# aapo-kossi/gym-eldorado

Hardware: AMD Instinct MI355X
Metric: env-steps/sec at n_envs=65536, 4 players; bit-exact vs C++ ref (higher is better)
Workload: dtype u8; 1 GPU; C5: 65,536 envs in total over the ranks, 4 players, HARD, n_pieces=3, max_steps=100000, on-device masked sampler over selected_action_masks + step, persistent rollout kernel, every step's AoS outputs stored in HBM; n_envs_total=65536, n_envs_per_gpu=65536, seed=12345, parallelism=env-sharded x1 by index (runner.h:33-38 block split), no collectives

## Files before the change

### gym-eldorado_amd/csrc/cog_engine.hip

```cpp
#include <hip/hip_runtime.h>
#include <algorithm>
#include <cstdlib>
#include <cstring>

#include "cog_engine.h"
#include "cog_tables.h"
#include "cog_rng.h"

#define DEV __device__ __forceinline__

#ifdef COG_STAMPS
DEV unsigned long long stamp_clock() {
  unsigned long long t;
  __builtin_amdgcn_sched_barrier(0);
  asm volatile("s_memtime %0\n\ts_waitcnt lgkmcnt(0)" : "=s"(t) :: "memory");
  __builtin_amdgcn_sched_barrier(0);
  return t;
}
#define STAMP(s, k)                                                                          \
  do {                                                                                       \
    const unsigned long long t_ = stamp_clock();                                             \
    if ((s).stamps && (threadIdx.x & 63) == 0)                                               \
      (s).stamps[((size_t)blockIdx.x * (blockDim.x / 64) + threadIdx.x / 64) * 16 + (k)] = t_; \
  } while (0)
// ... 2972 lines not shown
    const uint32_t meta = g[3].w;
    const bool rec = live && (meta & kMetaValid);
    const int ag = (int)((meta >> 2) & 3u), na = (int)((meta >> 4) & 3u), na1 = (int)((meta >> 6) & 3u);
    if (rec) {
      uint32_t dm = 0;
#pragma unroll
      for (int k = 0; k < 7; k++) {
        if (ne4(dk[k], sel4_of(I, ag, k))) dm |= 1u << k;
#pragma unroll
        for (int p = 0; p < 4; p++) I.d[p][k] = sel4(ag == p, dk[k], I.d[p][k]);
      }
#pragma unroll
      for (int k = 0; k < 7; k++) D.slot[k][l] = sel4_of(I, na1, k);
      PH(6);
#ifndef COG_ABLATE_DUOSTORES
      uint8_t *ob = s.obs + i * COG_OBS_BYTES;
      s.info[i * COG_INFO_BYTES + COG_AGENT_INFO0 + COG_AGENT_INFO_STRIDE * ag] = (uint8_t)(meta >> 8);
      if (meta & kMetaMoved) reinterpret_cast<uint4 *>(s.priv + i)[2] = g[6];
#pragma unroll
      for (int k = 0; k < 3; k++) {
        if (ne4(g[k], shb[k])) reinterpret_cast<uint4 *>(ob + COG_OBS_PHASE)[k] = g[k];
        shb[k] = g[k];
      }
      uint8_t *deck = deck_ptr(s, i, ag);
#pragma unroll
      for (int k = 0; k < 7; k++)
        if ((dm >> k) & 1u) reinterpret_cast<uint4 *>(deck)[k] = dk[k];
      const MBits bs{g[3].x, g[3].y, g[3].z}, ba{g[4].x, g[4].y, g[4].z};
      store_mask_record(reinterpret_cast<uint4 *>(s.sel + i * COG_MASK_BYTES), bs, mask_diff_granules(bs, selb));
      selb = bs;
      store_mask_record(reinterpret_cast<uint4 *>(deck + COG_PD_MASK), ba, mask_diff_granules(ba, selm(stb, ag)));
      setm(stb, ag, ba);
      if (na != ag) {
        const MBits bn{g[5].x, g[5].y, g[5].z};
        store_mask_record(reinterpret_cast<uint4 *>(deck_ptr(s, i, na) + COG_PD_MASK), bn,
                          mask_diff_granules(bn, selm(stb, na)));
        setm(stb, na, bn);
      }
      reinterpret_cast<uint2 *>(av + i * COG_ACTION_BYTES)[0] = make_uint2(g[4].w, g[5].w);
#else
      asm volatile("" ::"v"(g[0].x ^ g[1].y ^ g[2].z ^ g[3].x ^ g[4].y ^ g[5].z ^ g[6].w ^ dm ^ dk[0].x ^ dk[6].w));
#endif
      if (!(meta & kMetaEnded)) {
        const uint32_t agent = meta >> 24;
        if (out & 0xffu) s.done[i] = 0;
        if (((out >> 8) & 0xffu) != agent) s.agent[i] = (uint8_t)agent;
        out = agent << 8;
      }
    }
    PH(13);
    __syncthreads();
    PH(7);
  }
  PH_FLUSH(s_glob);
}

template <int SRC>
__global__ void __launch_bounds__(128) k_env_rollout_duo(DevState s, int steps, uint32_t *__restrict__ rngs,
                                                         uint8_t *__restrict__ actions_out) {
  __shared__ DuoLds D;
  const int role = __builtin_amdgcn_readfirstlane((int)(threadIdx.x >> 6));
  park_list_clear_other(s);
  uid_tab_fill(D.tab);
  if (role == 0) {
#ifndef DUO_NOPRIO
    __builtin_amdgcn_s_setprio(3);
#endif
    duo_stepper<SRC>(D, s, steps, rngs);
  } else {
    duo_storer(D, s, steps, actions_out);
  }
}

constexpr int kTrioRingG = 3;
#ifndef COG_TRIO_DEPTH
#define COG_TRIO_DEPTH 8
#endif
constexpr int kTrioDepth = COG_TRIO_DEPTH;
constexpr int kTrioLead = 4;
#ifndef COG_TRIO_BLAG
#define COG_TRIO_BLAG 2
#endif
constexpr int kTrioBLag = COG_TRIO_BLAG;
enum TrioCnt : int { CNT_REC = 0, CNT_DRAW, CNT_STA, CNT_STB, CNT_PRE, CNT_FIN, CNT_ABORT, kTrioCnts };
constexpr uint32_t kTrioSpinLimit = 1u << 21;
struct TrioLds {
  uint2 img[4][5][64];
  uint4 ring[kTrioDepth][kTrioRingG][64];
  uint32_t srng[kTrioDepth][64];
  uint3 pre[kTrioLead][64];
  uint4 pl[4][64];
  uint4 heads[4][64];
  uint4 stbA[4][64];
  uint32_t wide[64];
  uint32_t flg[64];
  uint32_t cnt[kTrioCnts];
  UidEntry tab[kUidTab];
};
static_assert(sizeof(TrioLds) <= 54613, "three trio workgroups per CU (trio_pad_lds keeps two)");
static_assert((kTrioDepth & (kTrioDepth - 1)) == 0 && kTrioDepth >= 4, "ring slots: a power of two");

struct TrioCnt6 {
  uint32_t rec = 0, draw = 0, sta = 0, stb = 0, pre = 0, fin = 0, abort = 0;
};
DEV void cnt_read(const TrioLds &D, TrioCnt6 &c) {
  uint32_t v[kTrioCnts];
#pragma unroll
  for (int k = 0; k < kTrioCnts; k++) v[k] = __hip_atomic_load(&D.cnt[k], __ATOMIC_RELAXED, __HIP_MEMORY_SCOPE_WORKGROUP);
  __builtin_amdgcn_fence(__ATOMIC_ACQUIRE, "workgroup");
  c.rec = __builtin_amdgcn_readfirstlane(v[CNT_REC]);
  c.draw = __builtin_amdgcn_readfirstlane(v[CNT_DRAW]);
  c.sta = __builtin_amdgcn_readfirstlane(v[CNT_STA]);
  c.stb = __builtin_amdgcn_readfirstlane(v[CNT_STB]);
  c.pre = __builtin_amdgcn_readfirstlane(v[CNT_PRE]);
  c.fin = __builtin_amdgcn_readfirstlane(v[CNT_FIN]);
  c.abort = __builtin_amdgcn_readfirstlane(v[CNT_ABORT]);
}
DEV void cnt_store(TrioLds &D, int k, uint32_t v) {
#ifdef COG_TRIO_FENCE
  if ((threadIdx.x & 63) == 0) __hip_atomic_store(&D.cnt[k], v, __ATOMIC_RELEASE, __HIP_MEMORY_SCOPE_WORKGROUP);
#else
  __builtin_amdgcn_fence(__ATOMIC_RELEASE, "wavefront");
  if ((threadIdx.x & 63) == 0) __hip_atomic_store(&D.cnt[k], v, __ATOMIC_RELAXED, __HIP_MEMORY_SCOPE_WORKGROUP);
  __builtin_amdgcn_fence(__ATOMIC_ACQUIRE, "wavefront");
#endif
}
#ifdef COG_ISSUE_COUNT
DEV void cnt_wait(TrioLds &, TrioCnt6 &, const uint32_t &field, uint32_t v, const DevState &) {
  if (field < v) asm volatile("s_nop 0");
}
#else
DEV void cnt_wait(TrioLds &D, TrioCnt6 &c, const uint32_t &field, uint32_t v, const DevState &s) {
  if (__builtin_expect(field >= v, 1)) return;
  if (c.abort) return;
  for (uint32_t spins = 0;; spins++) {
    cnt_read(D, c);
    if (field >= v || c.abort) return;
    if (spins >= kTrioSpinLimit) {
      if ((threadIdx.x & 63) == 0) {
        atomicOr(&s.status[0], F_SYNC_TIMEOUT);
        atomicAdd(&s.status[1], 1u);
        *s.err = 1u;
        __hip_atomic_store(&D.cnt[CNT_ABORT], 1u, __ATOMIC_RELEASE, __HIP_MEMORY_SCOPE_WORKGROUP);
      }
      c.abort = 1u;
      return;
    }
    __builtin_amdgcn_s_sleep(2);
  }
}
#endif
DEV uint3 pre_pack(const uint4 p, bool jtab) {
  if (!jtab) return make_uint3(p.x, p.y, p.z | p.w << 31);
  uint32_t jt = 0u;
#pragma unroll
  for (int k = 2; k <= 9; k++) {
    const UidEntry e = uid_entry((uint32_t)k);
    jt |= uid_tab_accepted(p.y, e.s, e.m) << (4 * (k - 2));
  }
  return make_uint3(p.x, jt, p.z | p.w << 31);
}

DEV void trio_store_players(const TrioLds &D, const DevState &s, int ne) {
  const int l = (int)(threadIdx.x & 63);
#pragma unroll
  for (int j = 0; j < 4; j++) {
    const int f = j * 64 + l, e = min(f >> 2, ne - 1), q = f & 3;
    reinterpret_cast<uint4 *>(s.priv + e)[4 + q] = D.pl[q][e];
    s.heads[5 * e + 1 + q] = D.heads[q][e];
  }
}

DEV void deck_expand(const uint2 pile[5], uint4 dk[7]) {
  uint32_t d[28];
#pragma unroll
  for (int k = 0; k < 28; k++) d[k] = 0u;
#pragma unroll
  for (int p = 0; p < 5; p++) {
    const int b = 21 * p, q = b >> 2, sh = b & 3;
    const uint32_t lo = pile[p].x, hi = pile[p].y;
    if (sh == 0) {
      d[q] |= lo;
      d[q + 1] |= hi;
    } else {
      d[q] |= lo << (8 * sh);
      d[q + 1] |= __builtin_amdgcn_alignbyte(hi, lo, 4 - sh);
      d[q + 2] |= hi >> (8 * (4 - sh));
    }
  }
#pragma unroll
  for (int k = 0; k < 7; k++) dk[k] = make_uint4(d[4 * k], d[4 * k + 1], d[4 * k + 2], d[4 * k + 3]);
}
DEV bool compact_of(const uint4 dk[7], uint2 pile[5]) {
  uint32_t d[28];
#pragma unroll
  for (int k = 0; k < 7; k++) { d[4 * k] = dk[k].x; d[4 * k + 1] = dk[k].y; d[4 * k + 2] = dk[k].z; d[4 * k + 3] = dk[k].w; }
  uint32_t rest = 0u;
#pragma unroll
  for (int k = 0; k < 28; k++) {
    uint32_t m = 0u;
#pragma unroll
    for (int y = 4 * k; y < 4 * k + 4; y++)
      if (y < 105 && y % 21 >= 8) m |= 0xffu << (8 * (y & 3));
    if (m) rest |= d[k] & m;
  }
#pragma unroll
  for (int p = 0; p < 5; p++) {
    const int b = 21 * p, q = b >> 2, sh = b & 3;
    pile[p].x = sh ? __builtin_amdgcn_alignbyte(d[q + 1], d[q], sh) : d[q];
    pile[p].y = sh ? __builtin_amdgcn_alignbyte(d[q + 2], d[q + 1], sh) : d[q + 1];
  }
  return rest == 0u;
}
DEV uint32_t hand_take(uint2 &h, int c) {
  const uint32_t sh = 8u * (uint32_t)(c & 3);
  const uint32_t w = c < 4 ? h.x : h.y;
  const uint32_t prev = (w >> sh) & 0xffu;
  const uint32_t nw = (w & ~(0xffu << sh)) | (((prev - 1u) & 0xffu) << sh);
  h.x = c < 4 ? nw : h.x;
  h.y = c < 4 ? h.y : nw;
  return prev;
}
DEV bool heads14_zero(const MBits &b) { return (b.w0 >> 22) == 1u && b.w1 == (1u << 12) && b.w2 == 0x204u; }
constexpr uint32_t kMoveShopBits = (0x7fu << 2) | (0x7ffffu << 9);
DEV uint32_t nth_set_bit_iter(uint32_t m, uint32_t j) {
  while (__builtin_amdgcn_ballot_w64(j != 0u)) {
    m = j ? (m & (m - 1u)) : m;
    j = j ? j - 1u : 0u;
  }
  return (uint32_t)(__ffs(m) - 1);
}
DEV bool sample_lean(const MBits &sel, const uint3 &pr, uint32_t &rng, uint32_t &a0, bool jtab, const UidEntry *tab) {
  const uint32_t m0 = sel.w0 & 0x3fffffu, k0 = __popc(m0);
  if (!(pr.x == rng && (pr.z >> 31) == 0u && heads14_zero(sel) && k0 >= 1u && k0 <= 9u)) return false;
  uint32_t j;
  if (jtab) {
    j = k0 >= 2u ? (pr.y >> (4u * (k0 - 2u))) & 15u : 0u;
  } else {
    const UidEntry e0 = tab[k0];
    j = k0 >= 2u ? uid_tab_accepted(pr.y, e0.s, e0.m) : 0u;
  }
  a0 = nth_set_bit_iter(m0, j);
  rng = pr.z;
  return true;
}
DEV uint4 pack_lean_player(uint4 pp, uint32_t n_in_hand, uint32_t n_active, uint32_t steps_taken) {
  pp.y = (pp.y & 0xff0000ffu) | (n_in_hand & 0xffu) << 8 | (n_active & 0xffu) << 16;
  pp.z = (pp.z & 0xffff00ffu) | (steps_taken & 0xffu) << 8;
  return pp;
}
DEV bool lean_player(const uint4 &pp) { return (pp.x | (pp.y & 0xffu)) == 0u; }
DEV void trio_store_private(const DevState &s, size_t i, const RegEnv &R, const MBits &selb) {
  uint4 *pw = reinterpret_cast<uint4 *>(s.priv + i);
  reinterpret_cast<uint3 *>(reinterpret_cast<uint32_t *>(pw) + 1)[0] = make_uint3(R.seed, R.max_steps, R.turn_counter);
  pw[1] = make_uint4(R.g1x, R.g1y, R.in_market, R.flags);
  s.heads[5 * i] = mbits_u4(selb);
}

template <int SRC, bool LAT>
DEV void trio_stepper(TrioLds &D, const DevState &s_glob, int steps, int epw, uint32_t *__restrict__ rngs_glob) {
  const int l = (int)(threadIdx.x & 63);
  const size_t wbase = (size_t)blockIdx.x * epw;
  const DevState s = wave_view(s_glob, wbase);
  const size_t i = (size_t)l;
  const int ne = (int)min((size_t)epw, s_glob.n - wbase);
  uint32_t *__restrict__ rngs = rngs_glob + wbase;
  bool live = l < ne;
  uint32_t park = kParkNone, srng = 0;
  PH_DECL;
  TL(10);
  RegEnv R;
  uint2 cells[4];
  int te1 = -1, te2 = -1;
  int ag = 0, na = 0;
  MBits selb = {0u, 0u, 0u}, stab = selb, stnb = selb;
  constexpr bool lat = LAT;
  uint4 pp = make_uint4(0u, 0u, 0u, 0u);
  uint32_t n_in_hand = 0u, n_active = 0u, steps_taken = 0u;
  uint32_t own = 0u;
  if (live) {
    Snap S;
    load_env(s, i, S);
    regs_env(R, S);
    const uint4 *pv4 = reinterpret_cast<const uint4 *>(s.priv + i);
#pragma unroll
    for (int p = 0; p < 4; p++) {
      D.pl[p][l] = pv4[4 + p];
      cells[p] = reinterpret_cast<const uint2 *>(pv4 + 8)[p];
      D.heads[p][l] = s.heads[5 * i + 1 + p];
    }
    srng = rngs[i];
    ag = (int)R.agent();
    na = (int)next_player((uint32_t)ag, R.n_players());
    pp = D.pl[ag][l];
    n_in_hand = (pp.y >> 8) & 0xffu;
    n_active = (pp.y >> 16) & 0xffu;
    steps_taken = (pp.z >> 8) & 0xffu;
#pragma unroll
    for (int p = 0; p < 4; p++) own |= (cells[p].x & 0xffu) << (8 * p);
    selb = S.sel;
    stab = mbits_of(D.heads[ag][l]);
    stnb = mbits_of(D.heads[na][l]);
  }
  R.tab = D.tab;
  __builtin_amdgcn_s_waitcnt(0);
  TL(15);
  __syncthreads();
  uint2 H = make_uint2(0u, 0u);
  bool lean_p = false, narrow = false;
  if (live) {
    H = D.img[ag][1][l];
    narrow = D.wide[l] == 0u;
    lean_p = narrow && lean_player(pp);
  }
  PH(6);
  TL(11);
  TrioCnt6 cc;
  uint3 pr_next = D.pre[0][l];
  bool have_next = true;
  uint2 pf_hd = make_uint2(0u, 0u);
  uint4 pf_pla = make_uint4(0u, 0u, 0u, 0u), pf_hdn = pf_pla;
  bool pf_ok = false;
  for (int t = 0; t < steps; t++) {
    const int sl = t & (kTrioDepth - 1);
    if (t >= kTrioDepth) {
      cnt_wait(D, cc, cc.sta, (uint32_t)(t - kTrioDepth + 1), s_glob);
      cnt_wait(D, cc, cc.stb, (uint32_t)(t - kTrioDepth + 1), s_glob);
    }
    PH(9);
    if (!have_next) cnt_wait(D, cc, cc.pre, (uint32_t)(t - kTrioLead + 1), s_glob);
    PH(2);
    bool ended = false, finish = false, turn_end = false, stepped = false;
    uint32_t a_play = 0u;
    {
      const uint32_t srng0 = srng;
      uint3 pr = pr_next;
      if (!have_next) pr = D.pre[t & (kTrioLead - 1)][l];
      const uint32_t m0 = selb.w0 & 0x3fffffu, k0 = __popc(m0);
      const bool fast = live && pr.x == srng && (pr.z >> 31) == 0u && heads14_zero(selb) && k0 - 1u < 9u;
      uint32_t j;
      if (LAT) {
        j = (pr.y >> (4u * ((k0 - 2u) & 7u))) & 15u;
      } else {
        const UidEntry e0 = R.tab[k0 & (kUidTab - 1)];
        j = uid_tab_accepted(pr.y, e0.s, e0.m);
      }
      j = fast && k0 >= 2u ? j : 0u;
      const uint32_t a0 = nth_set_bit_iter(m0, j);
      a_play = fast ? a0 : 0u;
      srng = fast ? pr.z : srng;
      bool other = false;
      if (__builtin_amdgcn_ballot_w64(live && !fast) && live && !fast) {
#ifdef COG_ISSUE_COUNT
        other = true;
#else
        uint8_t act[5];
        R.sel = heads_of(selb);
        step_action<SRC>(R, make_uint2(0u, 0u), srng, act);
        a_play = act[0];
        other = ((uint32_t)act[1] | act[2] | act[3] | act[4]) != 0u;
#endif
      }
      other = other || a_play > 8u;
      const bool was_done = R.done() != 0u;
      bool hook = false;
      if (t == s.redo_at) hook = s.redo_env < 0 || (int)(wbase + i) == s.redo_env;
      const bool parks = live && !was_done && (!lean_p || other || hook);
      stepped = live && !was_done && !parks;
      if (__builtin_amdgcn_ballot_w64(parks) && parks) {
        srng = srng0;
#ifndef COG_ISSUE_COUNT
        trio_store_private(s, i, R, selb);
        rngs[i] = srng;
#endif
        if (!lat) D.pl[ag][l] = pack_lean_player(pp, n_in_hand, n_active, steps_taken);
        park = (uint32_t)t | kParkRedo;
        live = false;
      }
      uint32_t phase = R.sh[0] & 0xffu;
      if (phase == COG_PHASE_INACTIVE) phase = COG_PHASE_MOVEMENT;
      if (!lat) steps_taken = stepped ? (steps_taken + 1u) & 0xffu : steps_taken;
      const bool play = stepped && a_play != 0u;
      const int c = (int)((a_play - 1u) & 7u);
      uint2 Hp = H;
      const uint32_t prev = hand_take(Hp, c);
      H = play ? Hp : H;
      const uint32_t bp = 1u << (c + 1);
      selb.w0 = play ? (prev > 1u ? (selb.w0 | bp) : (selb.w0 & ~bp)) : selb.w0;
      if (!lat) {
        n_in_hand = play ? (n_in_hand - 1u) & 0xffu : n_in_hand;
        n_active = play ? (n_active + 1u) & 0xffu : n_active;
        pp.z = play ? (pp.z & ~0xffu) | (uint32_t)c : pp.z;
      }
      const uint32_t nph = phase == COG_PHASE_BUYING ? COG_PHASE_INACTIVE : phase + 1u;
      phase = stepped && !play ? nph : phase;
      turn_end = stepped && phase == COG_PHASE_INACTIVE;
      n_active = turn_end ? 0u : n_active;
      const MBits sel0 = selb;
      selb.w0 = turn_end ? stnb.w0 : selb.w0;
      selb.w1 = turn_end ? stnb.w1 : selb.w1;
      selb.w2 = turn_end ? stnb.w2 : selb.w2;
      stab.w0 = turn_end ? sel0.w0 : stab.w0;
      stab.w1 = turn_end ? sel0.w1 : stab.w1;
      stab.w2 = turn_end ? sel0.w2 : stab.w2;
      stnb.w2 = turn_end ? (stnb.w2 & ~kMoveShopBits) | 0x204u : stnb.w2;
      R.g1y = turn_end ? (R.g1y & ~0xffu) | ((uint32_t)na & 0xffu) : R.g1y;
      R.turn_counter += turn_end ? 1u : 0u;
      R.sh[0] = stepped ? (R.sh[0] & ~0xffu) | phase : R.sh[0];
      finish = turn_end && (COG_HEX_END((own >> (8 * na)) & 0xffu) || R.turn_counter >= R.max_steps);
      R.g1x = finish ? (R.g1x & 0x00ffffffu) | (1u << 24) : R.g1x;
      PH(0);
      ended = live && (was_done || finish);
    }
    uint4(*ring)[64] = D.ring[sl];
    int ag1 = ag, na1 = na;
    if (live) {
      ag1 = (int)R.agent();
      na1 = (int)next_player((uint32_t)ag1, R.n_players());
    }
    const bool tc = live && ag1 != ag;
    const bool slow = tc && !pf_ok;
    if (__builtin_amdgcn_ballot_w64(slow)) {
      const int need = R.n_players() == 3u ? te1 : te2;
      const int needw = slow && need >= 0 ? need : INT32_MIN;
      if (__builtin_amdgcn_ballot_w64(needw >= 0)) {
        int dmin = 5;
#pragma unroll
        for (int d = 4; d >= 1; d--) dmin = __builtin_amdgcn_ballot_w64(needw >= t - d) ? d : dmin;
        PH(4);
        cnt_wait(D, cc, cc.draw, (uint32_t)(t - dmin + 1), s_glob);
        PH(5);
      }
      if (slow) {
        pf_hd = D.img[ag1][1][l];
        pf_pla = D.pl[ag1][l];
        pf_hdn = D.heads[na1][l];
      }
    }
    if (live) {
      if (!lat && (tc || ended)) D.pl[ag][l] = pack_lean_player(pp, n_in_hand, n_active, steps_taken);
      const uint32_t meta = kMetaValid | (uint32_t)ag << 2 | (uint32_t)na << 4 | (uint32_t)na1 << 6 |
                            (ended ? kMetaEnded : 0u) | (stepped ? kMetaStepped : 0u) | (uint32_t)ag1 << 24;
      ring[0][l].x = R.sh[0];
      ring[1][l] = make_uint4(selb.w0, selb.w1, selb.w2, meta);
      ring[2][l] = make_uint4(stab.w0, stab.w1, stab.w2, a_play | (lat ? 0u : (n_active & 0xffu) << 8));
      D.srng[sl][l] = srng;
    } else {
      ring[1][l] = make_uint4(0u, 0u, 0u, 0u);
    }
    cnt_store(D, CNT_REC, (uint32_t)(t + 1));
    have_next = t + 1 < kTrioLead || cc.pre >= (uint32_t)(t + 2 - kTrioLead);
    if (have_next) pr_next = D.pre[(t + 1) & (kTrioLead - 1)][l];
    PH(1);
    if (tc) {
      te2 = te1;
      te1 = t;
      H = pf_hd;
      pp = pf_pla;
      n_in_hand = (pf_pla.y >> 8) & 0xffu;
      n_active = (pf_pla.y >> 16) & 0xffu;
      steps_taken = (pf_pla.z >> 8) & 0xffu;
      lean_p = narrow && lean_player(pf_pla);
      stab = stnb;
      stnb = mbits_of(pf_hdn);
      pf_ok = false;
    }
    if (live && !pf_ok && !ended) {
      const int need = R.n_players() == 3u ? te1 : te2;
      if (need < 0 || cc.draw >= (uint32_t)(need + 1)) {
        const int nn = (int)next_player((uint32_t)na1, R.n_players());
        pf_hd = D.img[na1][1][l];
        pf_pla = D.pl[na1][l];
        pf_hdn = D.heads[nn][l];
        pf_ok = true;
      }
    }
    if (live && ended) {
#ifndef COG_ISSUE_COUNT
      trio_store_private(s, i, R, selb);
      rngs[i] = srng;
#endif
      park = (uint32_t)t | (finish ? kParkFinish : 0u);
      live = false;
    }
    ag = ag1;
    na = na1;
    PH(3);
  }
  TL(12);
  if (live && !lat) D.pl[ag][l] = pack_lean_player(pp, n_in_hand, n_active, steps_taken);
  cnt_store(D, CNT_REC, (uint32_t)steps + 1u);
  uint4 *pw = reinterpret_cast<uint4 *>(s.priv + i);
  if (lat) {
    if (live) {
      reinterpret_cast<uint3 *>(reinterpret_cast<uint32_t *>(pw) + 1)[0] = make_uint3(R.seed, R.max_steps, R.turn_counter);
      s.heads[5 * i] = mbits_u4(selb);
      rngs[i] = srng;
    }
    if (l < ne) s.park[i] = park;
    park_list_push(s_glob, park != kParkNone);
  }
  cnt_wait(D, cc, cc.fin, 3u, s_glob);
  PH(7);
  TL(13);
  const uint32_t fl = D.flg[l];
  if (lat) {
    if (live) pw[1] = make_uint4(R.g1x, R.g1y, R.in_market, R.flags | fl);
    else if (l < ne && fl) reinterpret_cast<uint32_t *>(pw)[7] = R.flags | fl;
  } else {
    if (live) {
      R.flags |= fl;
      trio_store_private(s, i, R, selb);
      rngs[i] = srng;
    } else if (l < ne && fl) {
      reinterpret_cast<uint32_t *>(pw)[7] = R.flags | fl;
    }
    if (l < ne) s.park[i] = park;
    park_list_push(s_glob, park != kParkNone);
  }
  trio_store_players(D, s, ne);
  PH(8);
  TL(14);
  PH_FLUSH(s_glob);
}

template <bool LAT>
DEV void trio_draw_play(TrioLds &D, const DevState &s, int l, bool live, int slot, uint32_t mt, uint32_t w2,
                        uint32_t gx, uint4 &p4, uint2 &h, uint2 &a, uint4 &shb0, uint32_t &infob, bool &te,
                        bool &rec_out, uint32_t &dm, uint32_t &nact) {
  const size_t i = (size_t)l;
  const int ag = (int)((mt >> 2) & 3u);
  const bool valid = live && (mt & kMetaValid);
  const bool rec = valid && (mt & kMetaStepped);
  rec_out = rec;
  te = rec && (int)(mt >> 24) != ag;
  const uint32_t a_play = w2 & 0xffu;
  const bool play = rec && a_play != 0u;
  const int c = (int)((a_play - 1u) & 7u);
  if (LAT) {
    uint4 q = p4;
    uint32_t na = (q.y >> 16) & 0xffu;
    q.z = (q.z & 0xffff00ffu) | (((q.z >> 8) + 1u) & 0xffu) << 8;
    q.y = play ? (q.y & 0xffff00ffu) | ((((q.y >> 8) & 0xffu) - 1u) & 0xffu) << 8 : q.y;
    na = play ? (na + 1u) & 0xffu : na;
    q.z = play ? (q.z & ~0xffu) | (a_play - 1u) : q.z;
    na = te ? 0u : na;
    q.y = (q.y & 0xff00ffffu) | na << 16;
    p4.x = rec ? q.x : p4.x;
    p4.y = rec ? q.y : p4.y;
    p4.z = rec ? q.z : p4.z;
    if (rec) D.pl[ag][l] = p4;
    nact = rec ? na : 0u;
  }
  infob = rec ? (infob & ~(0xffu << (8 * ag))) | ((((infob >> (8 * ag)) + 1u) & 0xffu) << (8 * ag)) : infob;
  uint32_t phase = shb0.x & 0xffu;
  phase = phase == COG_PHASE_INACTIVE ? (uint32_t)COG_PHASE_MOVEMENT : phase;
  const bool mv = play && phase == COG_PHASE_MOVEMENT, buy = play && phase == COG_PHASE_BUYING;
  const uint32_t coin = cardf(kRes2, c);
  uint4 g0 = shb0;
  g0.y = mv ? __float_as_uint((float)cardf(kRes0, c)) : g0.y;
  g0.z = mv ? __float_as_uint((float)cardf(kRes1, c)) : g0.z;
  const float bw = __uint_as_float(g0.w) + (coin > 0 ? (float)coin : 0.5f);
  g0.w = mv ? __float_as_uint((float)coin) : buy ? __float_as_uint(bw) : g0.w;
  g0.y = te ? 0u : g0.y;
  g0.z = te ? 0u : g0.z;
  g0.w = te ? 0u : g0.w;
  g0.x = rec ? gx : g0.x;
  if (valid) {
    reinterpret_cast<uint3 *>(&D.ring[slot][0][l].y)[0] = make_uint3(g0.y, g0.z, g0.w);
    s.info[i * COG_INFO_BYTES + COG_AGENT_INFO0 + COG_AGENT_INFO_STRIDE * ag] = (uint8_t)(infob >> (8 * ag));
    if (ne4(g0, shb0)) reinterpret_cast<uint4 *>(s.obs + i * COG_OBS_BYTES + COG_OBS_PHASE)[0] = g0;
  }
  shb0.x = valid ? g0.x : shb0.x;
  shb0.y = valid ? g0.y : shb0.y;
  shb0.z = valid ? g0.z : shb0.z;
  shb0.w = valid ? g0.w : shb0.w;
  const uint32_t sh = 8u * (uint32_t)(c & 3);
  uint32_t hw = c < 4 ? h.x : h.y, aw = c < 4 ? a.x : a.y;
  hw = (hw & ~(0xffu << sh)) | ((((hw >> sh) - 1u) & 0xffu) << sh);
  aw = (aw & ~(0xffu << sh)) | ((((aw >> sh) + 1u) & 0xffu) << sh);
  const bool lo = c < 4;
  h.x = play && lo ? hw : h.x;
  h.y = play && !lo ? hw : h.y;
  a.x = play && lo ? aw : a.x;
  a.y = play && !lo ? aw : a.y;
  if (play) {
    D.img[ag][1][l] = h;
    D.img[ag][2][l] = a;
  }
  const int bh = COG_DECK_HAND + c, ba = COG_DECK_ACTIVE + c;
  dm = play ? 1u << (bh >> 4) | 1u << (ba >> 4) : 0u;
}

template <bool LAT>
DEV uint32_t trio_drawer(TrioLds &D, const DevState &s_glob, int steps, int epw) {
  PH_DECL;
  TL(14);
  const int l = (int)(threadIdx.x & 63);
  const size_t wbase = (size_t)blockIdx.x * epw;
  const DevState s = wave_view(s_glob, wbase);
  const size_t i = (size_t)l;
  const bool live = l < epw && wbase + (size_t)l < s_glob.n;
  uint32_t rng = 0u;
  bool narrow = true;
  constexpr bool lat = LAT;
  uint4 shb0 = make_uint4(0u, 0u, 0u, 0u);
  uint32_t infob = 0u;
  if (live && !s_glob.cdeck_ok) {
#pragma unroll
    for (int p = 0; p < 4; p++) {
      const uint4 *src = reinterpret_cast<const uint4 *>(deck_ptr(s, i, p));
      uint4 dk[7];
      uint2 pile[5];
#pragma unroll
      for (int k = 0; k < 7; k++) dk[k] = src[k];
      narrow = compact_of(dk, pile) && narrow;
#pragma unroll
      for (int q = 0; q < 5; q++) D.img[p][q][l] = pile[q];
    }
  }
  if (live) {
    rng = reinterpret_cast<const uint32_t *>(s.priv + i)[0];
    infob = reinterpret_cast<const uint32_t *>(s.priv + i)[12];
    shb0 = reinterpret_cast<const uint4 *>(s.obs + i * COG_OBS_BYTES + COG_OBS_PHASE)[0];
  }
  if (!s_glob.cdeck_ok) D.wide[l] = narrow ? 0u : 1u;
  uint32_t flags = 0u;
  __builtin_amdgcn_s_waitcnt(0);
  TL(15);
  __syncthreads();
  PH_RESET;
  TrioCnt6 cc;
  for (int r = 0; r < steps; r += 2) {
    const int nrec = r + 1 < steps ? 2 : 1;
    cnt_wait(D, cc, cc.rec, (uint32_t)(r + nrec), s_glob);
    PH(8);
    if (r + nrec >= steps) TL(11);
    const int slot[2] = {r & (kTrioDepth - 1), (r + 1) & (kTrioDepth - 1)};
    uint32_t dm[2] = {0u, 0u}, nact[2] = {0u, 0u};
    int agj[2] = {0, 0};
    bool te[2] = {false, false}, recj[2] = {false, false};
    const uint32_t mt0 = D.ring[slot[0]][1][l].w, w20 = D.ring[slot[0]][2][l].w, gx0 = D.ring[slot[0]][0][l].x;
    uint32_t mt1 = D.ring[slot[1]][1][l].w;
    const uint32_t w21 = D.ring[slot[1]][2][l].w, gx1 = D.ring[slot[1]][0][l].x;
    if (nrec < 2) mt1 = 0u;
    const int ag0 = (int)((mt0 >> 2) & 3u), ag1 = (int)((mt1 >> 2) & 3u);
    uint4 p0 = make_uint4(0u, 0u, 0u, 0u), p1 = p0;
    if (lat) {
      p0 = D.pl[ag0][l];
      p1 = D.pl[ag1][l];
    }
    uint2 h0 = D.img[ag0][1][l], a0 = D.img[ag0][2][l], h1 = D.img[ag1][1][l], a1 = D.img[ag1][2][l];
    trio_draw_play<lat>(D, s, l, live, slot[0], mt0, w20, gx0, p0, h0, a0, shb0, infob, te[0], recj[0], dm[0], nact[0]);
    agj[0] = ag0;
    if (nrec > 1) {
      if (ag1 == ag0) {
        p1.x = p0.x; p1.y = p0.y; p1.z = p0.z; p1.w = p0.w;
        h1.x = h0.x; h1.y = h0.y;
        a1.x = a0.x; a1.y = a0.y;
      }
      trio_draw_play<lat>(D, s, l, live, slot[1], mt1, w21, gx1, p1, h1, a1, shb0, infob, te[1], recj[1], dm[1], nact[1]);
      agj[1] = ag1;
    }
    PH(7);
    const bool any = te[0] || te[1];
    if (__builtin_amdgcn_ballot_w64(any) && any) {
      const int j = te[1] ? 1 : 0, sl = te[1] ? slot[1] : slot[0], ag = te[1] ? agj[1] : agj[0];
      uint2 pile[5];
#pragma unroll
      for (int q = 0; q < 5; q++) pile[q] = D.img[ag][q][l];
      uint4 dk[7], old[7];
      deck_expand(pile, dk);
#pragma unroll
      for (int k = 0; k < 7; k++) old[k] = dk[k];
      const uint4 x = D.ring[sl][2][l];
      MBits ba{x.x, x.y, x.z};
      duo_turn_end(D, l, ag, dk, ba, rng, flags);
      D.ring[sl][2][l] = make_uint4(ba.w0, ba.w1, ba.w2, x.w);
      uint32_t dd = 0;
#pragma unroll
      for (int k = 0; k < 7; k++) dd |= ne4(dk[k], old[k]) ? 1u << k : 0u;
      (void)compact_of(dk, pile);
#pragma unroll
      for (int q = 0; q < 5; q++) D.img[ag][q][l] = pile[q];
      dm[0] |= j == 0 ? dd : 0u;
      dm[1] |= j == 1 ? dd : 0u;
    }
#pragma unroll
    for (int j = 0; j < 2; j++)
      if (j < nrec) {
        uint32_t *w = &D.ring[slot[j]][2][l].w;
        if (lat && recj[j]) *w = (*w & 0xffu) | nact[j] << 8 | dm[j] << 16;
        else reinterpret_cast<uint16_t *>(w)[1] = (uint16_t)dm[j];
      }
    cnt_store(D, CNT_DRAW, (uint32_t)(r + nrec));
    PH(9);
  }
  TL(12);
  if (live) {
    reinterpret_cast<uint32_t *>(s.priv + i)[0] = rng;
    reinterpret_cast<uint32_t *>(s.priv + i)[12] = infob;
  }
  PH_FLUSH(s_glob);
  return flags;
}

template <int PART, bool LAT>
DEV uint32_t trio_storer(TrioLds &D, const DevState &s_glob, int steps, int epw, const uint32_t *__restrict__ rngs_glob,
                         uint8_t *__restrict__ actions_glob) {
  PH_DECL;
  TL(14);
  const int l = (int)(threadIdx.x & 63);
  const size_t wbase = (size_t)blockIdx.x * epw;
  const DevState s = wave_view(s_glob, wbase);
  const size_t i = (size_t)l;
  const bool live = l < epw && wbase + (size_t)l < s_glob.n;
  uint8_t *__restrict__ av = actions_glob + wbase * COG_ACTION_BYTES;
  MBits selb = {0u, 0u, 0u};
  uint2 cells[4];
  uint32_t out = ~0u;
  RegEnv E;
  E.flags = 0u;
  E.avail = 0u;
  uint32_t x = 1u;
  if (live) {
    if (PART == 0) {
      const uint4 *sh4 = reinterpret_cast<const uint4 *>(s.obs + i * COG_OBS_BYTES + COG_OBS_PHASE);
      const uint4 sh1 = sh4[1], sh2 = sh4[2];
      const uint4 *pv4 = reinterpret_cast<const uint4 *>(s.priv + i);
#pragma unroll
      for (int p = 0; p < 4; p++) {
        D.stbA[p][l] = s.heads[5 * i + 1 + p];
        cells[p] = reinterpret_cast<const uint2 *>(pv4 + 8)[p];
      }
      const uint4 g1 = pv4[1];
      const uint32_t w[5] = {sh1.x, sh1.y, sh1.z, sh1.w, sh2.x};
      E.avail = shop_avail_of(w, (g1.y >> 8) & 0xffu, g1.z);
      if (s_glob.cdeck_ok) {
        const uint4 *src = s.cdeck + 10 * i;
        uint4 c[10];
#pragma unroll
        for (int g = 0; g < 10; g++) c[g] = src[g];
#pragma unroll
        for (int g = 0; g < 10; g++) {
          D.img[(2 * g) / 5][(2 * g) % 5][l] = make_uint2(c[g].x, c[g].y);
          D.img[(2 * g + 1) / 5][(2 * g + 1) % 5][l] = make_uint2(c[g].z, c[g].w);
        }
      }
    } else {
      selb = mbits_of(s.heads[5 * i]);
      x = rngs_glob[wbase + (size_t)l];
    }
  }
  if (PART == 0 && s_glob.cdeck_ok) D.wide[l] = live ? s.cwide[i] : 0u;
  if (PART == 1) {
#pragma unroll
    for (int k = 0; k < kTrioLead; k++) {
      const uint4 p = presample(x);
      D.pre[k][l] = pre_pack(p, LAT);
      x = p.z;
    }
  }
  __builtin_amdgcn_s_waitcnt(0);
  TL(15);
  __syncthreads();
  PH_RESET;
  constexpr int LAG = PART == 1 ? kTrioBLag : 0;
  auto deck_rec = [&](int q) {
    const int sl = q & (kTrioDepth - 1);
    const uint32_t meta = D.ring[sl][1][l].w;
    const int ag = (int)((meta >> 2) & 3u);
    if (live && (meta & kMetaValid)) {
      const uint32_t dm = D.ring[sl][2][l].w >> 16;
      uint2 pile[5];
#pragma unroll
      for (int k = 0; k < 5; k++) pile[k] = D.img[ag][k][l];
      uint4 dk[7];
      deck_expand(pile, dk);
      uint4 *deck = reinterpret_cast<uint4 *>(deck_ptr(s, i, ag));
#pragma unroll
      for (int k = 0; k < 7; k++)
        if ((dm >> k) & 1u) deck[k] = dk[k];
    }
    cnt_store(D, CNT_STB, (uint32_t)(q + 1));
  };
  TrioCnt6 cc;
  for (int r = 0; r < steps + LAG; r++) {
    if (PART == 1 && r < steps) {
      const int sl = r & (kTrioDepth - 1);
      cnt_wait(D, cc, cc.rec, (uint32_t)(r + 1), s_glob);
      PH(5);
      const uint4 m = D.ring[sl][1][l];
      const uint32_t meta = m.w;
      const bool rec = live && (meta & kMetaValid);
      if (rec && r + kTrioLead < steps)
        D.pre[(r + kTrioLead) & (kTrioLead - 1)][l] = pre_pack(presample(mr_jump(D.srng[sl][l], kPow15)), LAT);
      cnt_store(D, CNT_PRE, (uint32_t)(r + 1));
      const uint32_t a_play = D.ring[sl][2][l].w & 0xffu;
      if (rec) {
        const MBits bs{m.x, m.y, m.z};
        store_mask_record(reinterpret_cast<uint4 *>(s.sel + i * COG_MASK_BYTES), bs, mask_diff_granules(bs, selb));
        selb = bs;
        reinterpret_cast<uint2 *>(av + i * COG_ACTION_BYTES)[0] = make_uint2(a_play, 0u);
        if (!(meta & kMetaEnded)) {
          const uint32_t agent = meta >> 24;
          if (out & 0xffu) s.done[i] = 0;
          if (((out >> 8) & 0xffu) != agent) s.agent[i] = (uint8_t)agent;
          out = agent << 8;
        }
      }
    }
    PH(7);
    const int q = r - LAG;
    if (q < 0) continue;
    const int sl = q & (kTrioDepth - 1);
    cnt_wait(D, cc, cc.draw, (uint32_t)(q + 1), s_glob);
    PH(6);
    if (q == steps - 1) TL(11);
    const uint32_t meta = D.ring[sl][1][l].w;
    const bool rec = live && (meta & kMetaValid);
    const int ag = (int)((meta >> 2) & 3u), na = (int)((meta >> 4) & 3u);
    if (rec && PART == 0) {
      const uint4 g0 = D.ring[sl][0][l], xa = D.ring[sl][2][l], oa = D.stbA[ag][l];
      MBits ba{xa.x, xa.y, xa.z};
      if ((int)(meta >> 24) == ag && (meta & kMetaStepped)) {
        const uint32_t phase = g0.x & 0xffu;
        const float r0 = __uint_as_float(g0.y), r1 = __uint_as_float(g0.z), r2 = __uint_as_float(g0.w);
        const uint32_t n_active = (xa.w >> 8) & 0xffu;
        uint2 ca = cells[3];
#pragma unroll
        for (int p = 2; p >= 0; p--) ca = ag == p ? cells[p] : ca;
        const uint32_t mv = phase == COG_PHASE_MOVEMENT ? E.move_bits(ca, r0, r1, r2, n_active) : 1u;
        const uint32_t sp = phase == COG_PHASE_BUYING ? E.shop_bits(r2) : 1u;
        ba.w2 = (ba.w2 & ~kMoveShopBits) | mv << 2 | sp << 9;
      }
      uint8_t *deck = deck_ptr(s, i, ag);
      store_mask_record(reinterpret_cast<uint4 *>(deck + COG_PD_MASK), ba, mask_diff_granules(ba, mbits_of(oa)));
      D.stbA[ag][l] = mbits_u4(ba);
      if ((int)(meta >> 24) != ag && (meta & kMetaStepped)) {
        const uint4 on = D.stbA[na][l];
        const MBits bn{on.x, on.y, (on.z & ~kMoveShopBits) | 0x204u};
        store_mask_record(reinterpret_cast<uint4 *>(deck_ptr(s, i, na) + COG_PD_MASK), bn,
                          mask_diff_granules(bn, mbits_of(on)));
        D.stbA[na][l] = mbits_u4(bn);
      }
    }
    if (PART == 1) {
      deck_rec(q);
    } else {
      cnt_store(D, CNT_STA, (uint32_t)(q + 1));
    }
    PH(13);
  }
  TL(12);
  if (PART == 0) {
    cnt_wait(D, cc, cc.rec, (uint32_t)steps + 1u, s_glob);
    if (live) {
#pragma unroll
      for (int p = 0; p < 4; p++) D.heads[p][l] = D.stbA[p][l];
      uint4 *dst = s.cdeck + 10 * i;
#pragma unroll
      for (int g = 0; g < 10; g++) {
        const uint2 a = D.img[(2 * g) / 5][(2 * g) % 5][l], b = D.img[(2 * g + 1) / 5][(2 * g + 1) % 5][l];
        dst[g] = make_uint4(a.x, a.y, b.x, b.y);
      }
      s.cwide[i] = D.wide[l];
    }
  }
  PH_FLUSH(s_glob);
  return E.flags;
}

template <int SRC, bool LAT>
__global__ void __launch_bounds__(256) __attribute__((amdgpu_waves_per_eu(4))) k_env_rollout_trio(DevState s, int steps, int epw, uint32_t *__restrict__ rngs,
                                                          uint8_t *__restrict__ actions_out) {
  __shared__ TrioLds D;
  const int role = __builtin_amdgcn_readfirstlane((int)(threadIdx.x >> 6));
  if (threadIdx.x < 64) D.flg[threadIdx.x] = 0u;
  if (threadIdx.x < kTrioCnts) D.cnt[threadIdx.x] = 0u;
  park_list_clear_other(s);
  uid_tab_fill(D.tab);
  if (role == 0) {
    __builtin_amdgcn_s_setprio(3);
    trio_stepper<SRC, LAT>(D, s, steps, epw, rngs);
    return;
  }
  uint32_t flags;
  if (role == 1) flags = trio_drawer<LAT>(D, s, steps, epw);
  else if (role == 2) flags = trio_storer<0, LAT>(D, s, steps, epw, rngs, actions_out);
  else flags = trio_storer<1, LAT>(D, s, steps, epw, rngs, actions_out);
  const int l = (int)(threadIdx.x & 63);
  if (flags) __hip_atomic_fetch_or(&D.flg[l], flags, __ATOMIC_RELAXED, __HIP_MEMORY_SCOPE_WORKGROUP);
  if (l == 0) __hip_atomic_fetch_add(&D.cnt[CNT_FIN], 1u, __ATOMIC_RELEASE, __HIP_MEMORY_SCOPE_WORKGROUP);
}
// ... 48 lines not shown
    uint32_t rng = rngs[i];
    uint8_t a[5];
    sample_mask(masks + i * COG_MASK_BYTES, rng, a, tab);
    rngs[i] = rng;
    store_action(actions + i * COG_ACTION_BYTES, a);
    if (h_actions) store_action(h_actions + i * COG_ACTION_BYTES, a);
  }
  grid_signal(sig);
}

constexpr unsigned kPublishPerItem = 2, kPublishSignalBlocks = 128;
__global__ void __launch_bounds__(256) k_publish(const uint4 *__restrict__ obs, const uint4 *__restrict__ outs,
                                                 uint4 *__restrict__ mir, uint4 *__restrict__ h_obs,
                                                 uint4 *__restrict__ h_outs, size_t n, size_t outs_g, int force,
                                                 const uint2 *__restrict__ act, uint2 *__restrict__ h_act,
                                                 GridSignal sig) {
  const size_t tail = n * kTailG, ng = tail + outs_g;
  const size_t t0 = ((size_t)blockIdx.x * blockDim.x) * kPublishPerItem + threadIdx.x;
  const uint4 *src[kPublishPerItem];
  uint4 *dst[kPublishPerItem];
  uint4 c[kPublishPerItem], m[kPublishPerItem];
  bool cmp[kPublishPerItem];
#pragma unroll
  for (unsigned j = 0; j < kPublishPerItem; j++) {
    const size_t t = t0 + (size_t)j * blockDim.x;
    src[j] = nullptr;
    if (t < tail) {
      const size_t row = t / kTailG, a = row * kRecG + kTail0 + (t - kTailG * row);
      src[j] = obs + a;
      dst[j] = h_obs + a;
      cmp[j] = !force;
    } else if (t < ng) {
      const size_t u = t - tail;
      src[j] = outs + u;
      dst[j] = h_outs + u;
      cmp[j] = !force && u >= 4;
    }
    if (src[j]) {
      c[j] = *src[j];
      if (cmp[j]) m[j] = mir[t];
    }
  }
#pragma unroll
  for (unsigned j = 0; j < kPublishPerItem; j++) {
    const size_t t = t0 + (size_t)j * blockDim.x;
    if (src[j] && (!cmp[j] || ne4(c[j], m[j]))) {
      *dst[j] = c[j];
      mir[t] = c[j];
    }
  }
  const size_t ia = (size_t)blockIdx.x * blockDim.x + threadIdx.x;
  const size_t g_items = (ng + kPublishPerItem - 1) / kPublishPerItem;
  if (act && ia >= g_items && ia - g_items < n) {
    const size_t i = ia - g_items;
    h_act[(COG_ACTION_BYTES / 8) * i] = act[(COG_ACTION_BYTES / 8) * i];
  }
  grid_signal(sig);
}

__global__ void k_sync_heads(DevState s) {
  const size_t i = (size_t)blockIdx.x * blockDim.x + threadIdx.x;
  if (i < s.n) sync_heads(s, i);
}
__global__ void k_resync(DevState s) {
  const size_t i = (size_t)blockIdx.x * blockDim.x + threadIdx.x;
  if (i >= s.n) return;
  sync_heads(s, i);
  const uint8_t *inf = s.info + i * COG_INFO_BYTES + COG_AGENT_INFO0;
  uint32_t v = 0u;
#pragma unroll
  for (int p = 0; p < 4; p++) v |= (uint32_t)inf[COG_AGENT_INFO_STRIDE * p] << (8 * p);
  reinterpret_cast<uint32_t *>(s.priv + i)[12] = v;
}

__global__ void __launch_bounds__(64) k_signal(uint32_t *word, uint32_t seq) {
  if (threadIdx.x == 0) __hip_atomic_store(word, seq, __ATOMIC_RELEASE, __HIP_MEMORY_SCOPE_SYSTEM);
}

__global__ void k_seed_sampler(size_t n, uint64_t seed, size_t first, uint32_t *rngs) {
  const size_t i = (size_t)blockIdx.x * blockDim.x + threadIdx.x;
  if (i < n) rngs[i] = mr_seed(seed + (uint64_t)(first + i));
}

typedef unsigned int u32x4_t __attribute__((ext_vector_type(4)));
template <bool NT>
DEV u32x4_t cp_ld(const u32x4_t *p) {
  if (NT) return __builtin_nontemporal_load(p);
  return *p;
}
template <bool NT>
DEV void cp_st(u32x4_t v, u32x4_t *p) {
  if (NT) __builtin_nontemporal_store(v, p);
  else *p = v;
}
template <bool NT>
__global__ void __launch_bounds__(256) k_copy_peak(const u32x4_t *__restrict__ src, u32x4_t *__restrict__ dst, size_t n16) {
  const size_t stride = (size_t)gridDim.x * blockDim.x;
  size_t i = (size_t)blockIdx.x * blockDim.x + threadIdx.x;
  for (; i + 3 * stride < n16; i += 4 * stride) {
    const u32x4_t a = cp_ld<NT>(src + i), b = cp_ld<NT>(src + i + stride);
    const u32x4_t c = cp_ld<NT>(src + i + 2 * stride), d = cp_ld<NT>(src + i + 3 * stride);
    cp_st<NT>(a, dst + i);
    cp_st<NT>(b, dst + i + stride);
    cp_st<NT>(c, dst + i + 2 * stride);
    cp_st<NT>(d, dst + i + 3 * stride);
  }
  for (; i < n16; i += stride) cp_st<NT>(cp_ld<NT>(src + i), dst + i);
}
template <bool NT>
__global__ void __launch_bounds__(256) k_copy_block(const u32x4_t *__restrict__ src, u32x4_t *__restrict__ dst, size_t n16) {
  const size_t base = (size_t)blockIdx.x * 2048 + threadIdx.x;
  if (base + 7 * 256 < n16) {
    u32x4_t v[8];
#pragma unroll
    for (int k = 0; k < 8; k++) v[k] = cp_ld<NT>(src + base + k * 256);
#pragma unroll
    for (int k = 0; k < 8; k++) cp_st<NT>(v[k], dst + base + k * 256);
  } else {
    for (size_t i = base; i < n16; i += 256) cp_st<NT>(cp_ld<NT>(src + i), dst + i);
  }
}
template <bool NT>
__global__ void __launch_bounds__(256) k_copy_one(const u32x4_t *__restrict__ src, u32x4_t *__restrict__ dst, size_t n16) {
  const size_t i = (size_t)blockIdx.x * 256 + threadIdx.x;
  if (i < n16) cp_st<NT>(cp_ld<NT>(src + i), dst + i);
}

template <bool NT>
__global__ void __launch_bounds__(256) k_stream_mix(const u32x4_t *__restrict__ src, u32x4_t *__restrict__ dst, size_t n_rd) {
  const size_t i = (size_t)blockIdx.x * blockDim.x + threadIdx.x;
  if (i >= n_rd) return;
  const u32x4_t v = cp_ld<false>(src + i);
#pragma unroll
  for (int k = 0; k < 7; k++) cp_st<NT>(v + (unsigned)k, dst + i + (size_t)k * n_rd);
}

static inline unsigned blocks_for(size_t n, unsigned t) { return (unsigned)((n + t - 1) / t); }

int launch_init(const DevState &s, const uint32_t *, uint32_t default_seed, void *stream) {
  if (!s.n) return 0;
  hipLaunchKernelGGL(k_init, dim3(blocks_for(s.n, 256)), dim3(256), 0, (hipStream_t)stream, s, default_seed);
  hipLaunchKernelGGL(k_sync_heads, dim3(blocks_for(s.n, 256)), dim3(256), 0, (hipStream_t)stream, s);
  return hipGetLastError() == hipSuccess ? 0 : -1;
}
int launch_reset(const DevState &s, const ResetParams &p, void *stream) {
  if (!s.n) return 0;
  static const int epw_env = [] {
    const char *e = getenv("COG_RESET_EPW");
    return e ? atoi(e) : 0;
  }();
  const size_t auto_epw = (s.n + 4095) / 4096;
  const int epw = epw_env > 0 ? (epw_env < 64 ? epw_env : 64) : (int)(auto_epw < 1 ? 1 : auto_epw > 64 ? 64 : auto_epw);
  hipLaunchKernelGGL(k_reset, dim3(blocks_for(s.n, (unsigned)epw)), dim3(64), 0, (hipStream_t)stream, s, p, epw);
  hipLaunchKernelGGL(k_sync_heads, dim3(blocks_for(s.n, 256)), dim3(256), 0, (hipStream_t)stream, s);
  return hipGetLastError() == hipSuccess ? 0 : -1;
}
int launch_resync(const DevState &s, void *stream) {
  if (!s.n) return 0;
  hipLaunchKernelGGL(k_resync, dim3(blocks_for(s.n, 256)), dim3(256), 0, (hipStream_t)stream, s);
  return hipGetLastError() == hipSuccess ? 0 : -1;
}
int launch_encode_all(const DevState &s, void *stream, int variant) {
  if (!s.n) return 0;
  const size_t nb = s.n * kEncBlocks;
  const dim3 g(blocks_for(nb, 256)), b(256);
  if (variant == 1) hipLaunchKernelGGL(k_encode_lds<false>, g, b, 0, (hipStream_t)stream, s.cgrid, s.obs, nb);
  else if (variant == 2) hipLaunchKernelGGL(k_encode_direct, g, b, 0, (hipStream_t)stream, s.cgrid, s.obs, nb);
// ... 247 lines not shown
```

Before: 26.40 billion env-steps/s.

## Prefetch trio pipeline counters speculatively to cut LDS spin-wait latency

```diff
diff --git a/gym-eldorado_amd/csrc/cog_engine.hip b/gym-eldorado_amd/csrc/cog_engine.hip
--- a/gym-eldorado_amd/csrc/cog_engine.hip
+++ b/gym-eldorado_amd/csrc/cog_engine.hip
@@ -3078,7 +3078,7 @@
 #define COG_TRIO_BLAG 2
 #endif
 constexpr int kTrioBLag = COG_TRIO_BLAG;
-enum TrioCnt : int { CNT_REC = 0, CNT_DRAW, CNT_STA, CNT_STB, CNT_PRE, CNT_FIN, CNT_ABORT, kTrioCnts };
+enum TrioCnt : int { CNT_DRAW = 0, CNT_STA, CNT_STB, CNT_PRE, CNT_REC, CNT_FIN, CNT_ABORT, kTrioCnts };
 constexpr uint32_t kTrioSpinLimit = 1u << 21;
 struct TrioLds {
   uint2 img[4][5][64];
@@ -3090,14 +3090,19 @@
   uint4 stbA[4][64];
   uint32_t wide[64];
   uint32_t flg[64];
-  uint32_t cnt[kTrioCnts];
+  alignas(16) uint32_t cnt[8];
   UidEntry tab[kUidTab];
 };
 static_assert(sizeof(TrioLds) <= 54613, "three trio workgroups per CU (trio_pad_lds keeps two)");
 static_assert((kTrioDepth & (kTrioDepth - 1)) == 0 && kTrioDepth >= 4, "ring slots: a power of two");
 
 struct TrioCnt6 {
-  uint32_t rec = 0, draw = 0, sta = 0, stb = 0, pre = 0, fin = 0, abort = 0;
+  uint32_t rec = 0, draw = 0, sta = 0, stb = 0, pre = 0, fin = 0, abort = 0, ring = 0;
+#ifdef COG_CENSUS
+  uint32_t n_enter = 0, n_first = 0;
+  unsigned long long ticks = 0;
+  uint32_t n_pre = 0, n_ring = 0, ahead = 0;
+#endif
 };
 DEV void cnt_read(const TrioLds &D, TrioCnt6 &c) {
   uint32_t v[kTrioCnts];
@@ -3111,6 +3116,42 @@
   c.pre = __builtin_amdgcn_readfirstlane(v[CNT_PRE]);
   c.fin = __builtin_amdgcn_readfirstlane(v[CNT_FIN]);
   c.abort = __builtin_amdgcn_readfirstlane(v[CNT_ABORT]);
+  c.ring = min(c.sta, c.stb);
+}
+typedef unsigned int u32x4_t __attribute__((ext_vector_type(4)));
+DEV u32x4_t cnt_refresh(const TrioLds &D) {
+  __builtin_amdgcn_fence(__ATOMIC_RELEASE, "wavefront");
+  const u32x4_t v = *(const volatile __attribute__((address_space(3))) u32x4_t *)&D.cnt[0];
+  __builtin_amdgcn_fence(__ATOMIC_ACQUIRE, "wavefront");
+  return v;
+}
+DEV void cnt_harvest(TrioCnt6 &c, const u32x4_t v) {
+  c.draw = __builtin_amdgcn_readfirstlane(v[CNT_DRAW]);
+  c.sta = __builtin_amdgcn_readfirstlane(v[CNT_STA]);
+  c.stb = __builtin_amdgcn_readfirstlane(v[CNT_STB]);
+  c.pre = __builtin_amdgcn_readfirstlane(v[CNT_PRE]);
+  c.ring = min(c.sta, c.stb);
+#ifdef COG_TRIO_FENCE
+  __builtin_amdgcn_fence(__ATOMIC_ACQUIRE, "workgroup");
+#endif
+}
+struct TrioCntRaw {
+  uint32_t rec, draw;
+};
+DEV TrioCntRaw cnt_refresh_rd(const TrioLds &D) {
+  TrioCntRaw v;
+  __builtin_amdgcn_fence(__ATOMIC_RELEASE, "wavefront");
+  v.rec = __hip_atomic_load(&D.cnt[CNT_REC], __ATOMIC_RELAXED, __HIP_MEMORY_SCOPE_WORKGROUP);
+  v.draw = __hip_atomic_load(&D.cnt[CNT_DRAW], __ATOMIC_RELAXED, __HIP_MEMORY_SCOPE_WORKGROUP);
+  __builtin_amdgcn_fence(__ATOMIC_ACQUIRE, "wavefront");
+  return v;
+}
+DEV void cnt_harvest_rd(TrioCnt6 &c, const TrioCntRaw &v) {
+  c.rec = __builtin_amdgcn_readfirstlane(v.rec);
+  c.draw = __builtin_amdgcn_readfirstlane(v.draw);
+#ifdef COG_TRIO_FENCE
+  __builtin_amdgcn_fence(__ATOMIC_ACQUIRE, "workgroup");
+#endif
 }
 DEV void cnt_store(TrioLds &D, int k, uint32_t v) {
 #ifdef COG_TRIO_FENCE
@@ -3121,17 +3162,31 @@
   __builtin_amdgcn_fence(__ATOMIC_ACQUIRE, "wavefront");
 #endif
 }
+DEV bool cnt_has(uint32_t c, uint32_t v) { return (int32_t)(c - v) >= 0; }
 #ifdef COG_ISSUE_COUNT
 DEV void cnt_wait(TrioLds &, TrioCnt6 &, const uint32_t &field, uint32_t v, const DevState &) {
-  if (field < v) asm volatile("s_nop 0");
+  if (!cnt_has(field, v)) asm volatile("s_nop 0");
 }
 #else
 DEV void cnt_wait(TrioLds &D, TrioCnt6 &c, const uint32_t &field, uint32_t v, const DevState &s) {
-  if (__builtin_expect(field >= v, 1)) return;
+  if (__builtin_expect(cnt_has(field, v), 1)) return;
   if (c.abort) return;
+#ifdef COG_CENSUS
+  const unsigned long long census_t0 = stamp_clock();
+  c.n_enter++;
+#endif
   for (uint32_t spins = 0;; spins++) {
     cnt_read(D, c);
-    if (field >= v || c.abort) return;
+#ifdef COG_CENSUS
+    if (cnt_has(field, v) || c.abort) {
+      c.n_first += spins == 0u ? 1u : 0u;
+      c.ticks += stamp_clock() - census_t0;
+      c.n_pre += &field == &c.pre ? 1u : 0u;
+      c.n_ring += &field == &c.ring ? 1u : 0u;
+      c.ahead += spins == 0u ? field - v : 0u;
+    }
+#endif
+    if (cnt_has(field, v) || c.abort) return;
     if (spins >= kTrioSpinLimit) {
       if ((threadIdx.x & 63) == 0) {
         atomicOr(&s.status[0], F_SYNC_TIMEOUT);
@@ -3224,7 +3279,7 @@
     m = j ? (m & (m - 1u)) : m;
     j = j ? j - 1u : 0u;
   }
-  return (uint32_t)(__ffs(m) - 1);
+  return (uint32_t)__builtin_ctz(m);
 }
 DEV bool sample_lean(const MBits &sel, const uint3 &pr, uint32_t &rng, uint32_t &a0, bool jtab, const UidEntry *tab) {
   const uint32_t m0 = sel.w0 & 0x3fffffu, k0 = __popc(m0);
@@ -3313,19 +3368,18 @@
   TL(11);
   TrioCnt6 cc;
   uint3 pr_next = D.pre[0][l];
-  bool have_next = true;
+  uint32_t pre_seen = 0u;
   uint2 pf_hd = make_uint2(0u, 0u);
   uint4 pf_pla = make_uint4(0u, 0u, 0u, 0u), pf_hdn = pf_pla;
   bool pf_ok = false;
   for (int t = 0; t < steps; t++) {
     const int sl = t & (kTrioDepth - 1);
-    if (t >= kTrioDepth) {
-      cnt_wait(D, cc, cc.sta, (uint32_t)(t - kTrioDepth + 1), s_glob);
-      cnt_wait(D, cc, cc.stb, (uint32_t)(t - kTrioDepth + 1), s_glob);
-    }
+    cnt_wait(D, cc, cc.ring, (uint32_t)(t - kTrioDepth + 1), s_glob);
     PH(9);
-    if (!have_next) cnt_wait(D, cc, cc.pre, (uint32_t)(t - kTrioLead + 1), s_glob);
+    const bool have_next = cnt_has(pre_seen, (uint32_t)(t - kTrioLead + 1));
+    cnt_wait(D, cc, cc.pre, (uint32_t)(t - kTrioLead + 1), s_glob);
     PH(2);
+    u32x4_t cnt_hot;
     bool ended = false, finish = false, turn_end = false, stepped = false;
     uint32_t a_play = 0u;
     {
@@ -3333,7 +3387,8 @@
       uint3 pr = pr_next;
       if (!have_next) pr = D.pre[t & (kTrioLead - 1)][l];
       const uint32_t m0 = selb.w0 & 0x3fffffu, k0 = __popc(m0);
-      const bool fast = live && pr.x == srng && (pr.z >> 31) == 0u && heads14_zero(selb) && k0 - 1u < 9u;
+      const bool fast = live & (pr.x == srng) & ((pr.z >> 31) == 0u) & ((selb.w0 >> 22) == 1u) &
+                        (selb.w1 == (1u << 12)) & (selb.w2 == 0x204u) & (k0 - 1u < 9u);
       uint32_t j;
       if (LAT) {
         j = (pr.y >> (4u * ((k0 - 2u) & 7u))) & 15u;
@@ -3342,11 +3397,13 @@
         j = uid_tab_accepted(pr.y, e0.s, e0.m);
       }
       j = fast && k0 >= 2u ? j : 0u;
+      __builtin_amdgcn_sched_barrier(0);
+      cnt_hot = cnt_refresh(D);
       const uint32_t a0 = nth_set_bit_iter(m0, j);
       a_play = fast ? a0 : 0u;
       srng = fast ? pr.z : srng;
       bool other = false;
-      if (__builtin_amdgcn_ballot_w64(live && !fast) && live && !fast) {
+      if (live && !fast) {
 #ifdef COG_ISSUE_COUNT
         other = true;
 #else
@@ -3363,7 +3420,7 @@
       if (t == s.redo_at) hook = s.redo_env < 0 || (int)(wbase + i) == s.redo_env;
       const bool parks = live && !was_done && (!lean_p || other || hook);
       stepped = live && !was_done && !parks;
-      if (__builtin_amdgcn_ballot_w64(parks) && parks) {
+      if (parks) {
         srng = srng0;
 #ifndef COG_ISSUE_COUNT
         trio_store_private(s, i, R, selb);
@@ -3382,7 +3439,7 @@
       const uint32_t prev = hand_take(Hp, c);
       H = play ? Hp : H;
       const uint32_t bp = 1u << (c + 1);
-      selb.w0 = play ? (prev > 1u ? (selb.w0 | bp) : (selb.w0 & ~bp)) : selb.w0;
+      selb.w0 = (selb.w0 & ~(play ? bp : 0u)) | (play && prev > 1u ? bp : 0u);
       if (!lat) {
         n_in_hand = play ? (n_in_hand - 1u) & 0xffu : n_in_hand;
         n_active = play ? (n_active + 1u) & 0xffu : n_active;
@@ -3408,12 +3465,11 @@
       PH(0);
       ended = live && (was_done || finish);
     }
+    cnt_harvest(cc, cnt_hot);
+    pre_seen = cc.pre;
+    if (cnt_has(pre_seen, (uint32_t)(t + 2 - kTrioLead))) pr_next = D.pre[(t + 1) & (kTrioLead - 1)][l];
     uint4(*ring)[64] = D.ring[sl];
-    int ag1 = ag, na1 = na;
-    if (live) {
-      ag1 = (int)R.agent();
-      na1 = (int)next_player((uint32_t)ag1, R.n_players());
-    }
+    const int ag1 = (int)R.agent(), na1 = (int)next_player((uint32_t)ag1, R.n_players());
     const bool tc = live && ag1 != ag;
     const bool slow = tc && !pf_ok;
     if (__builtin_amdgcn_ballot_w64(slow)) {
@@ -3432,6 +3488,7 @@
         pf_pla = D.pl[ag1][l];
         pf_hdn = D.heads[na1][l];
       }
+      __builtin_amdgcn_s_waitcnt(0xc07f);
     }
     if (live) {
       if (!lat && (tc || ended)) D.pl[ag][l] = pack_lean_player(pp, n_in_hand, n_active, steps_taken);
@@ -3445,8 +3502,6 @@
       ring[1][l] = make_uint4(0u, 0u, 0u, 0u);
     }
     cnt_store(D, CNT_REC, (uint32_t)(t + 1));
-    have_next = t + 1 < kTrioLead || cc.pre >= (uint32_t)(t + 2 - kTrioLead);
-    if (have_next) pr_next = D.pre[(t + 1) & (kTrioLead - 1)][l];
     PH(1);
     if (tc) {
       te2 = te1;
@@ -3517,6 +3572,14 @@
   trio_store_players(D, s, ne);
   PH(8);
   TL(14);
+#ifdef COG_CENSUS
+  ph_.acc[10] = cc.n_enter;
+  ph_.acc[11] = cc.n_first;
+  ph_.acc[12] = cc.ticks;
+  ph_.acc[13] = cc.n_pre;
+  ph_.acc[14] = cc.n_ring;
+  ph_.acc[15] = cc.ahead;
+#endif
   PH_FLUSH(s_glob);
 }
 
@@ -3647,6 +3710,8 @@
       p1 = D.pl[ag1][l];
     }
     uint2 h0 = D.img[ag0][1][l], a0 = D.img[ag0][2][l], h1 = D.img[ag1][1][l], a1 = D.img[ag1][2][l];
+    TrioCntRaw cnt_rd = {0u, 0u};
+    if (!LAT) cnt_rd = cnt_refresh_rd(D);
     trio_draw_play<lat>(D, s, l, live, slot[0], mt0, w20, gx0, p0, h0, a0, shb0, infob, te[0], recj[0], dm[0], nact[0]);
     agj[0] = ag0;
     if (nrec > 1) {
@@ -3690,6 +3755,7 @@
         else reinterpret_cast<uint16_t *>(w)[1] = (uint16_t)dm[j];
       }
     cnt_store(D, CNT_DRAW, (uint32_t)(r + nrec));
+    if (!LAT) cnt_harvest_rd(cc, cnt_rd);
     PH(9);
   }
   TL(12);
@@ -3781,18 +3847,21 @@
     cnt_store(D, CNT_STB, (uint32_t)(q + 1));
   };
   TrioCnt6 cc;
+  TrioCntRaw cnt_rd = {0u, 0u};
   for (int r = 0; r < steps + LAG; r++) {
     if (PART == 1 && r < steps) {
       const int sl = r & (kTrioDepth - 1);
       cnt_wait(D, cc, cc.rec, (uint32_t)(r + 1), s_glob);
       PH(5);
       const uint4 m = D.ring[sl][1][l];
+      const uint32_t sr = D.srng[sl][l];
+      const uint32_t a_play = D.ring[sl][2][l].w & 0xffu;
       const uint32_t meta = m.w;
       const bool rec = live && (meta & kMetaValid);
+      if (!LAT) cnt_rd = cnt_refresh_rd(D);
       if (rec && r + kTrioLead < steps)
-        D.pre[(r + kTrioLead) & (kTrioLead - 1)][l] = pre_pack(presample(mr_jump(D.srng[sl][l], kPow15)), LAT);
+        D.pre[(r + kTrioLead) & (kTrioLead - 1)][l] = pre_pack(presample(mr_jump(sr, kPow15)), LAT);
       cnt_store(D, CNT_PRE, (uint32_t)(r + 1));
-      const uint32_t a_play = D.ring[sl][2][l].w & 0xffu;
       if (rec) {
         const MBits bs{m.x, m.y, m.z};
         store_mask_record(reinterpret_cast<uint4 *>(s.sel + i * COG_MASK_BYTES), bs, mask_diff_granules(bs, selb));
@@ -3806,6 +3875,7 @@
         }
       }
     }
+    if (!LAT && PART == 1 && r < steps) cnt_harvest_rd(cc, cnt_rd);
     PH(7);
     const int q = r - LAG;
     if (q < 0) continue;
@@ -4020,7 +4090,6 @@
   if (i < n) rngs[i] = mr_seed(seed + (uint64_t)(first + i));
 }
 
-typedef unsigned int u32x4_t __attribute__((ext_vector_type(4)));
 template <bool NT>
 DEV u32x4_t cp_ld(const u32x4_t *p) {
   if (NT) return __builtin_nontemporal_load(p);
```

Result: no change. 26.40 billion env-steps/s (-0.0%).
